# niksaz/aido1

Measured on AMD Instinct MI355X. Metric: env-steps/sec (whole node) at 4096 envs/GPU; pose/reward max-abs-err vs CPU ref, higher is better.
Workload: dtype f64 step / f32 raster + grey / u8 masks; 1 GPU; config3: 4096 envs/GPU, lane pose + 120x160 top-down render + grey frame ring + line_detector1 HSV/edge masks; map=loop_empty, envs_per_gpu=4096, global_envs=4096, repeat_actions=3, auto_reset=True, actions=U[0,1)^2 wheel velocities, resident in HBM, parallelism=env shards (1 x 4096), no collective

## Files before the change

aido1_amd/_lib.py:

```python
import ctypes
import os
import subprocess
import threading

from aido1_amd.config import DtConfig

PKG_DIR = os.path.dirname(os.path.abspath(__file__))
REPO_DIR = os.path.dirname(PKG_DIR)
LIB_PATH = os.path.join(PKG_DIR, 'libdtsim.so')
CSRC = os.path.join(PKG_DIR, 'csrc')
SOURCES = ['dtsim.hip', 'dtrender.hip', 'dtreplay.hip', 'dtactor.hip', 'dtconv.hip',
           'dtconvx.hip', 'dttrain.hip', 'dtupd.hip', 'dthead.hip']
HEADERS = ['dtsim_common.h', 'dtrender.h', 'dtsync.h', 'dtconv_common.h']
PUBLIC_HEADERS = ['dtsim.h', 'dtreplay.h', 'dtactor.h', 'dttrain.h', 'dtupd.h', 'dthead.h']
HIPCC = os.environ.get('HIPCC', '/opt/rocm/bin/hipcc')
ABI_VERSION = 14

HIP_FLAGS = ['--offload-arch=gfx950', '-O3', '-fPIC', '-shared', '-std=c++17',
             '-ffp-contract=off', '-munsafe-fp-atomics']
FILE_FLAGS = {'dtrender.hip': ['-fno-slp-vectorize']}


class DtError(RuntimeError):
    pass
# ... 83 lines not shown
                print(' '.join(cmd))

        def run(cmd):
            return subprocess.run(cmd, capture_output=True, text=True)
        with ThreadPoolExecutor(max_workers=min(8, len(jobs))) as ex:
            results = list(ex.map(run, [c for c, _ in jobs]))
        for (cmd, _), r in zip(jobs, results):
            if r.returncode != 0:
                raise DtError('hipcc failed building %s (%s):\n' % (
                    os.path.basename(path), os.path.basename(cmd[-3])) + r.stderr[-4000:])
        link = [HIPCC, '--offload-arch=gfx950', '-shared', '-fPIC', '-o', tmp] + \
            [o for _, o in jobs]
        if verbose:
            print(' '.join(link))
        r = subprocess.run(link, capture_output=True, text=True)
        if r.returncode != 0:
            raise DtError('hipcc failed linking %s:\n' % os.path.basename(path) + r.stderr[-4000:])
        os.replace(tmp, path)
    finally:
        shutil.rmtree(objdir, ignore_errors=True)
    return path


_OPTIONAL = set()

_lib = None
_lock = threading.Lock()


def bind(L):
    vp, i32, u32, u64 = ctypes.c_void_p, ctypes.c_int32, ctypes.c_uint32, ctypes.c_uint64
    i64, f64 = ctypes.c_int64, ctypes.c_double
    sig = {
        'dt_abi_version': (i32, []),
        'dt_create': (ctypes.c_int, [ctypes.POINTER(DtConfig), ctypes.POINTER(DtMap), u64, i32,
                                     i32, ctypes.POINTER(vp)]),
        'dt_destroy': (ctypes.c_int, [vp]),
        'dt_n_envs': (i32, [vp]),
        'dt_last_error': (ctypes.c_char_p, [vp]),
        'dt_seed': (ctypes.c_int, [vp, vp, u64, u32]),
        'dt_reset': (ctypes.c_int, [vp, vp, vp]),
        'dt_step': (ctypes.c_int, [vp, vp, vp, vp, vp, vp, vp, vp, vp]),
        'dt_step_masked': (ctypes.c_int, [vp, vp, vp, vp, vp, vp, vp, vp, vp, vp]),
        'dt_step_many': (ctypes.c_int, [vp, i32, vp, vp, vp, vp, vp, vp, vp]),
        'dt_seed_env': (ctypes.c_int, [vp, i32, u64]),
        'dt_lane_pos': (ctypes.c_int, [vp, vp, vp, vp]),
        'dt_render': (ctypes.c_int, [vp, vp, vp]),
        'dt_render2': (ctypes.c_int, [vp, vp, vp, vp]),
        'dt_render3': (ctypes.c_int, [vp, vp, vp, vp, vp]),
        'dt_copy_pose': (ctypes.c_int, [vp, vp, vp]),
        'dt_render_order': (ctypes.c_int, [vp, ctypes.POINTER(u32), vp, vp]),
        'dt_palette_gray': (ctypes.c_int, [ctypes.POINTER(ctypes.c_float)]),
        'dt_default_line_params': (ctypes.c_int, [vp]),
        'dt_set_line_params': (ctypes.c_int, [vp, vp]),
        'dt_line_detect': (ctypes.c_int, [vp, vp, i32, i32, i32, vp, vp, vp]),
        'dt_hough_lines': (ctypes.c_int, [vp, i32, i32, i32, i32, i32, i32, i32, vp, vp,
                                          vp]),
        'dt_line_detect_workspace': (ctypes.c_size_t, [i32, i32, i32]),
        'dt_line_detect_ws': (ctypes.c_int, [vp, vp, i32, i32, i32, vp, vp, vp,
                                             ctypes.c_size_t, vp]),
        'dt_hough_workspace': (ctypes.c_size_t, [i32, i32, i32]),
        'dt_hough_lines_ws': (ctypes.c_int, [vp, i32, i32, i32, i32, i32, i32, i32, vp, vp,
                                             vp, ctypes.c_size_t, vp]),
        'dt_get_state': (ctypes.c_int, [vp, vp, vp, vp, vp, vp, vp]),
        'dt_set_state': (ctypes.c_int, [vp, vp, vp, vp, vp, vp, vp]),
        'dt_check': (ctypes.c_int, [vp, ctypes.POINTER(u32)]),
        'dt_stats': (ctypes.c_int, [vp, ctypes.POINTER(ctypes.c_uint64), i32]),
        'dt_per_create': (ctypes.c_int, [i64, f64, i32, ctypes.POINTER(vp)]),
        'dt_per_destroy': (None, [vp]),
        'dt_per_last_error': (ctypes.c_char_p, [vp]),
        'dt_per_capacity': (i64, [vp]),
        'dt_per_len': (i64, [vp]),
        'dt_per_next_idx': (i64, [vp]),
        'dt_per_add': (ctypes.c_int, [vp, i64, vp, vp]),
        'dt_per_sample': (ctypes.c_int, [vp, i32, vp, f64, vp, vp, vp]),
# ... 149 lines not shown
```

aido1_amd/csrc/dthandle.h:

```cpp
#pragma once
#include <string>

#include "dtrender.h"
#include "dtsim_common.h"

struct StepCfg {
  int32_t repeat, frame_skip, action_mode, clip, speed_measured, auto_reset;
  uint32_t max_steps, max_env_steps, max_spawn_attempts;
  double reward_scale;
};

struct dt_handle {
  int device = 0;
  int n = 0;
  dt_config cfg{};
  dt::Geo geo{};
  StepCfg sc{};
  dt::MapDev map{};
  void* map_buf = nullptr;
  dt::State st{};
  void* st_buf = nullptr;
  size_t lds_bytes = 0;
  uint32_t env_base = 0;
  dt_line_params line_params{};
  dr::LineDev line{};
  void* mark_buf = nullptr;
  int32_t n_yellow = 0, n_white = 0;
  void* render_spill = nullptr;
  void* render_sched = nullptr;
  uint32_t render_launches = 0;
  hipEvent_t render_done = nullptr;
  hipStream_t render_stream = nullptr;
  bool render_pending = false;
  std::string err;
};

struct DevGuard {
  int prev = -1;
  explicit DevGuard(int device) {
    if (hipGetDevice(&prev) == hipSuccess && prev != device) {
      if (hipSetDevice(device) != hipSuccess) prev = -1;
    } else {
      prev = -1;
    }
  }
  ~DevGuard() {
    if (prev >= 0) (void)hipSetDevice(prev);
  }
  DevGuard(const DevGuard&) = delete;
  DevGuard& operator=(const DevGuard&) = delete;
// ... 16 lines not shown
```

aido1_amd/csrc/dtrender.h:

```cpp
#pragma once
#pragma clang fp contract(off)

#include <hip/hip_runtime.h>
#include <stdint.h>

#include "../../include/dtsim.h"

namespace dr {

constexpr int H = DT_OBS_H, W = DT_OBS_W, NPIX = H * W;
constexpr int kThreads = 256;
constexpr float kRes = 0.01f;
constexpr float kInvRes = 100.0f;

enum : uint8_t { PAL_FLOOR = 0, PAL_OFFROAD = 1, PAL_ROAD = 2, PAL_RED = 3, PAL_YELLOW = 4,
                 PAL_WHITE = 7, PAL_N = 8 };
__host__ __device__ constexpr uint32_t rgb_pack(uint32_t r, uint32_t g, uint32_t b) {
  return b | (g << 8) | (r << 16);
}
constexpr uint32_t kYellowRgb = rgb_pack(255, 230, 0);
constexpr uint32_t kPalette[PAL_N] = {
    rgb_pack(0, 0, 0),
    rgb_pack(72, 132, 52),
    rgb_pack(56, 56, 60),
// ... 71 lines not shown
  const int c0 = c > 0 ? c - 1 : 0, c2 = c < wid - 1 ? c + 1 : wid - 1;
  const uint32_t p00 = fetch(r0, c0), p01 = fetch(r0, c), p02 = fetch(r0, c2);
  const uint32_t p10 = fetch(r, c0), p12 = fetch(r, c2);
  const uint32_t p20 = fetch(r2, c0), p21 = fetch(r2, c), p22 = fetch(r2, c2);
  mag = -1;
  dx = dy = 0;
#pragma unroll
  for (int ch = 0; ch < 3; ++ch) {
    const int sh = 8 * ch;
    const int a00 = (p00 >> sh) & 255, a01 = (p01 >> sh) & 255, a02 = (p02 >> sh) & 255;
    const int a10 = (p10 >> sh) & 255, a12 = (p12 >> sh) & 255;
    const int a20 = (p20 >> sh) & 255, a21 = (p21 >> sh) & 255, a22 = (p22 >> sh) & 255;
    const int gx = (a02 + 2 * a12 + a22) - (a00 + 2 * a10 + a20);
    const int gy = (a20 + 2 * a21 + a22) - (a00 + 2 * a01 + a02);
    const int m = (gx < 0 ? -gx : gx) + (gy < 0 ? -gy : gy);
    if (m > mag) {
      mag = m;
      dx = gx;
      dy = gy;
    }
  }
}

__device__ inline uint8_t nms_dir(int dx, int dy) {
  constexpr int TG22 = 13573;
  const int x = dx < 0 ? -dx : dx;
  const int y = (dy < 0 ? -dy : dy) << 15;
  const int tg22x = x * TG22;
  if (y < tg22x) return 0;
  const int tg67x = tg22x + (x << 16);
  if (y > tg67x) return 1;
  return ((dx ^ dy) < 0) ? 3 : 2;
}

}
```

aido1_amd/csrc/dtrender.hip:

```cpp
#include <math.h>
#include <stdlib.h>
#include <string.h>

#include <vector>

#include "dthandle.h"

namespace {

using namespace dr;

#ifdef DTSIM_STAMPS
__device__ unsigned long long g_renstamps[4096 * 24];
__device__ inline unsigned ren_hw_id() {
  unsigned v;
  asm volatile("s_getreg_b32 %0, hwreg(HW_REG_HW_ID)" : "=s"(v));
  return v;
}
__device__ inline unsigned ren_xcc_id() {
  unsigned v;
  asm volatile("s_getreg_b32 %0, hwreg(HW_REG_XCC_ID)" : "=s"(v));
  return v;
}
#define RENSTAMP(i, v)                                                              \
// ... 45 lines not shown
        double dx, dz;
        bez_host(cp, (double)k / kSegs, px[k], pz[k], dx, dz);
        const double n = sqrt(dx * dx + dz * dz);
        rx[k] = (0.0 - dz) / n;
        rz[k] = dx / n;
      }
      for (int w = 0; w < kWhiteW; ++w) {
        const double o = kWhiteOff * ts + (2 * w - (kWhiteW - 1)) * kHalfStep;
        for (int k = 0; k < kSegs; ++k)
          white.push_back(make_float4((float)(px[k] + o * rx[k]), (float)(pz[k] + o * rz[k]),
                                      (float)(px[k + 1] + o * rx[k + 1]),
                                      (float)(pz[k + 1] + o * rz[k + 1])));
      }
      if (c != 0) continue;
      for (int w = 0; w < kYellowW; ++w) {
        const double o = kYellowOff * ts + (2 * w - (kYellowW - 1)) * kHalfStep;
        for (int k = 0; k < kSegs; k += 2)
          yellow.push_back(make_float4((float)(px[k] + o * rx[k]), (float)(pz[k] + o * rz[k]),
                                       (float)(px[k + 1] + o * rx[k + 1]),
                                       (float)(pz[k + 1] + o * rz[k + 1])));
      }
    }
  }
}

LineDev to_line_dev(const dt_line_params& p) {
  LineDev L{};
  memcpy(L.lo[0], p.hsv_white1, 3);
  memcpy(L.hi[0], p.hsv_white2, 3);
  memcpy(L.lo[1], p.hsv_yellow1, 3);
  memcpy(L.hi[1], p.hsv_yellow2, 3);
  memcpy(L.lo[2], p.hsv_red1, 3);
  memcpy(L.hi[2], p.hsv_red2, 3);
  memcpy(L.lo[3], p.hsv_red3, 3);
  memcpy(L.hi[3], p.hsv_red4, 3);
  const int k = p.dilation_kernel_size;
  const int r = k / 2;
  L.dil_r = r;
  L.dil_mask = 0;
  if (r == 0) {
    L.dil_mask = 1ull << (3 * 7 + 3);
  } else {
    const double inv_r2 = 1.0 / ((double)r * r);
    for (int i = 0; i < k; ++i) {
      const int dy = i - r;
      const int dxm = (int)lrint(r * sqrt((double)(r * r - dy * dy) * inv_r2));
// ... 105 lines not shown
      if (hyst_visit(S, hgt, wid, idx)) changed = 1;
    if (!__syncthreads_or(changed)) break;
  }
}

__device__ inline uint8_t pass_c_pixel(const PixBuf& S, const LineDev& L, int hgt, int wid, int r,
                                       int c) {
  uint8_t bits = 0;
  const int R = L.dil_r;
  for (int dy = -R; dy <= R; ++dy) {
    const int rr = r + dy;
    if ((unsigned)rr >= (unsigned)hgt) continue;
    for (int dx = -R; dx <= R; ++dx) {
      const int cc = c + dx;
      if ((unsigned)cc >= (unsigned)wid) continue;
      if (!((L.dil_mask >> ((dy + 3) * 7 + (dx + 3))) & 1ull)) continue;
      bits |= S.work[rr * wid + cc] & 7;
    }
  }
  if (S.work[r * wid + c] & B_EDGE) bits |= 8;
  return bits;
}

struct View {
  float cx, cz, dirx, dirz, rx, rz;
};

__device__ __forceinline__ int opaque_tid() {
  int t = (int)threadIdx.x;
#if DTSIM_RENDER_SEQ
  asm volatile("" : "+v"(t));
#endif
  return t;
}

#ifndef DTSIM_RENDER_SEQ
#define DTSIM_RENDER_SEQ 0
#endif
struct RenderArgs {
  const double* x;
  const double* z;
  const double* angle;
  const int8_t* kind;
  int32_t width, height;
  float inv_ts;
  double cam_fwd;
  const float4* marks;
  int32_t n_yellow, n_white;
  float* gray;
  uint8_t* index;
  int32_t slots, slot;
  const uint8_t* fresh;
  uint8_t* masks;
  uint8_t* rgb;
  uint16_t* spill;
  int32_t list_cap;
  LineDev line;
  int32_t n;
  uint32_t* sched;
  uint32_t launch;
  int32_t parts;
  int32_t slot2, slot3;
  const double* pose2;
  const double* pose3;
  const uint8_t* fresh2;
  const uint8_t* fresh3;
  uint8_t* masks2;
  uint8_t* masks3;
};

#ifndef DTSIM_MARK_PARTS
#define DTSIM_MARK_PARTS 2
#endif
#ifndef DTSIM_RENDER_THREADS
#define DTSIM_RENDER_THREADS 512
#endif
constexpr int kRenderThreads = DTSIM_RENDER_THREADS;
#ifdef DTSIM_RENDER_STOP_AT
#define RENDER_STOP(k) \
  if ((k) == DTSIM_RENDER_STOP_AT) return
#else
#define RENDER_STOP(k)
#endif
constexpr int WPR = W / 4;
constexpr int NW = NPIX / 4;
constexpr int QPR = WPR / 4;
constexpr int NQ = NW / 4;
constexpr int kListCap = 1984;
constexpr int kWeakCap = 512;
constexpr int kSegRecs = 2176;
constexpr int kSpillHalves = 5 * NW;
enum { kNSpan = 0, kNSeg = 1, kNList = 2, kNQuad = 3, kNWeak = 4, kNCnt = 8 };
constexpr uint16_t WK_MAG = 0x7FF, WK_DIR_SHIFT = 11, WK_CAND = 1 << 14, WK_EDGE = 1 << 15;

struct RenderLds {
  uint32_t img[NW];
  union {
    struct {
      uint16_t ent[4 * kListCap];
      uint16_t list[kListCap];
    } w;
    struct {
      uint2 seg[kSegRecs];
      uint16_t qlist[NQ];
    } p;
  } u;
  uint16_t weak[kWeakCap];
  uint32_t pal_swar[PAL_N];
  float pal_gray[PAL_N];
  uint32_t bits_lo, bits_hi;
  View view[3];
  int32_t cnt[kNCnt];
  int32_t env;
// ... 102 lines not shown

__device__ inline void wave_slots4(int32_t* counter, const bool want[4], int slot[4]) {
  wave_slotsN<4>(counter, want, slot);
}

__device__ inline int wave_slot1(int32_t* counter, bool want) {
  const uint64_t b = __ballot(want);
  if (b == 0) return 0;
  int base = 0;
  if ((threadIdx.x & 63) == 0) base = atomicAdd(counter, __popcll(b));
  base = __builtin_amdgcn_readlane(base, 0);
  return base + lane_prefix(b);
}

__device__ inline void wave_push4(int32_t* counter, uint16_t* list, int cap, const bool want[4],
                                  const uint16_t value[4]) {
  int slot[4];
  wave_slots4(counter, want, slot);
#pragma unroll
  for (int k = 0; k < 4; ++k)
    if (want[k] && slot[k] < cap) list[slot[k]] = value[k];
}

__device__ inline void wave_slots4x2(int32_t* counter, const bool wa[4], const bool wb[4],
                                     int sa[4], int sb[4]) {
  const uint32_t ca = (uint32_t)wa[0] + wa[1] + wa[2] + wa[3];
  const uint32_t cb = (uint32_t)wb[0] + wb[1] + wb[2] + wb[3];
  const uint64_t a0 = __ballot(ca & 1u), a1 = __ballot(ca & 2u), a2 = __ballot(ca & 4u);
  const uint64_t b0 = __ballot(cb & 1u), b1 = __ballot(cb & 2u), b2 = __ballot(cb & 4u);
  const uint32_t ta = __popcll(a0) + 2 * __popcll(a1) + 4 * __popcll(a2);
  const uint32_t tb = __popcll(b0) + 2 * __popcll(b1) + 4 * __popcll(b2);
  if ((ta | tb) == 0u) return;
  int base = 0;
  if ((threadIdx.x & 63) == 0) base = atomicAdd(counter, (int)(ta | (tb << 16)));
  base = __builtin_amdgcn_readlane(base, 0);
  int na = (base & 0xFFFF) + lane_prefix(a0) + 2 * lane_prefix(a1) + 4 * lane_prefix(a2);
  int nb = (int)((uint32_t)base >> 16) + lane_prefix(b0) + 2 * lane_prefix(b1) +
           4 * lane_prefix(b2);
#pragma unroll
  for (int k = 0; k < 4; ++k) {
    sa[k] = na;
    na += wa[k] ? 1 : 0;
    sb[k] = nb;
    nb += wb[k] ? 1 : 0;
  }
}

using lds_u32 = __attribute__((address_space(3))) uint32_t;

__device__ __forceinline__ void or_pixel(lds_u32* img, uint32_t ad, uint32_t col) {
  __hip_atomic_fetch_or(img + (ad >> 2), col << (8 * (ad & 3u)), __ATOMIC_RELAXED,
                        __HIP_MEMORY_SCOPE_WORKGROUP);
}

__device__ inline void draw_line_part(lds_u32* img, int x0, int y0, int x1, int y1, uint32_t col,
                                      int part, int parts) {
  int dx = x1 - x0, dy = y1 - y0;
  const int xsign = dx > 0 ? 1 : -1, ysign = dy > 0 ? 1 : -1;
  dx = dx < 0 ? -dx : dx;
  dy = dy < 0 ? -dy : dy;
  int xx, xy, yx, yy;
  if (dx > dy) {
    xx = xsign; xy = 0; yx = 0; yy = ysign;
  } else {
    const int t = dx; dx = dy; dy = t;
    xx = 0; xy = ysign; yx = xsign; yy = 0;
  }
  const int n = dx + 1;
  const int xa = (n * part) / parts, xb = (n * (part + 1)) / parts;
  if (xa >= xb) return;
  const int ya = dx > 0 ? (int)floorf((float)(2 * dy * xa + dx) / (float)(2 * dx)) : 0;
  int D = 2 * dy * (xa + 1) - dx - 2 * dx * ya;
  int px = x0 + xa * xx + ya * yx, py = y0 + xa * xy + ya * yy;
  int ad = py * W + px;
  const int amaj = xy * W + xx, amin = yy * W + yx;
  for (int x = xa; x < xb; ++x) {
    if ((unsigned)px < (unsigned)W && (unsigned)py < (unsigned)H) or_pixel(img, (uint32_t)ad, col);
    const bool st = D >= 0;
    px += xx + (st ? yx : 0);
    py += xy + (st ? yy : 0);
    ad += amaj + (st ? amin : 0);
    D += 2 * dy - (st ? 2 * dx : 0);
  }
}

__device__ inline int proj(float v) {
  v = floorf(v + 0.5f);
  v = v < -100000.0f ? -100000.0f : (v > 100000.0f ? 100000.0f : v);
  return (int)v;
}

__device__ inline bool project_seg(const View& V, float4 q, int& c0, int& r0, int& c1, int& r1) {
  const float ax = q.x - V.cx, az = q.y - V.cz, bx = q.z - V.cx, bz = q.w - V.cz;
  const float fa = ax * V.dirx + az * V.dirz, la = ax * V.rx + az * V.rz;
  const float fb = bx * V.dirx + bz * V.dirz, lb = bx * V.rx + bz * V.rz;
  c0 = proj(la * kInvRes + 79.5f);
  r0 = proj(119.5f - fa * kInvRes);
  c1 = proj(lb * kInvRes + 79.5f);
  r1 = proj(119.5f - fb * kInvRes);
  if ((c0 < 0 && c1 < 0) || (c0 >= W && c1 >= W) || (r0 < 0 && r1 < 0) || (r0 >= H && r1 >= H))
    return false;
  const int len = (c1 > c0 ? c1 - c0 : c0 - c1) + (r1 > r0 ? r1 - r0 : r0 - r1);
  return len <= 400;
}

__device__ inline uint2 seg_pack(int c0, int r0, int c1, int r1) {
  return make_uint2((uint32_t)(uint16_t)c0 | ((uint32_t)(uint16_t)r0 << 16),
                    (uint32_t)(uint16_t)c1 | ((uint32_t)(uint16_t)r1 << 16));
}

__device__ inline void seg_draw(lds_u32* img, uint2 v, uint32_t col, int part, int parts) {
  draw_line_part(img, (int)(int16_t)(v.x & 0xFFFFu), (int)(int16_t)(v.x >> 16),
                 (int)(int16_t)(v.y & 0xFFFFu), (int)(int16_t)(v.y >> 16), col, part, parts);
}

__device__ __forceinline__ uint32_t bg_color(const RenderLds& S, const RenderArgs& a, float fi,
                                             float fj) {
  if (fi >= 0.0f && fj >= 0.0f && fi < (float)a.width && fj < (float)a.height) {
    const int k = S.kind[__mul24((int)fj, a.width) + (int)fi];
    return k > 0 ? PAL_ROAD : (k == 0 ? PAL_OFFROAD : PAL_FLOOR);
  }
  return PAL_FLOOR;
}

__device__ inline View view_of(double x, double z, double ang, double cam_fwd) {
  double sd, cd;
// ... 441 lines not shown

__device__ __forceinline__ uint32_t sched_builder(const RenderArgs& a) {
#if DTSIM_RENDER_SEQ
  return (uint32_t)(a.n - kSchedTail);
#else
  return (uint32_t)(a.parts * a.n - kSchedTail);
#endif
}

__device__ __forceinline__ void sched_exit(const RenderArgs& a, RenderLds& S, int e) {
  if (threadIdx.x == 0) {
    const unsigned long long dt = __builtin_amdgcn_s_memtime() - S.t0;
    __hip_atomic_store(sched_cost(a) + e, dt > 0xFFFFFFFFull ? 0xFFFFFFFFu : (uint32_t)dt,
                       __ATOMIC_RELAXED, __HIP_MEMORY_SCOPE_AGENT);
  }
  if (blockIdx.x == sched_builder(a) && a.n <= kSchedMaxN) {
    __syncthreads();
    sched_build(a, S, a.launch);
  }
}

template <bool kIdx, bool kBigR>
__device__ __forceinline__ void render_env(const RenderArgs& a, RenderLds& S, int e, int half,
                                           int vi
#ifdef DTSIM_EARLY_MARKS
                                           , const float4 (&mq)[4]
#endif
) {
  const int tid = opaque_tid();
  constexpr int T = kRenderThreads;
  const LineDev& L = a.line;
  const int nmark = a.n_yellow + a.n_white;
  const bool mfast = nmark <= kMarkFast;
#ifdef DTSIM_STAMPS
  RENSTAMP(0, __builtin_amdgcn_s_memrealtime());
  RENSTAMP(2, ren_hw_id());
  RENSTAMP(3, ren_xcc_id());
#endif
  RENT(4);
  int32_t* const C = S.cnt;
  const View V = S.view[vi];
  lds_u32* const img = (lds_u32*)S.img;
#ifndef DTSIM_EARLY_MARKS
  float4 mq[4];
  if (mfast) {
#pragma unroll
    for (int k = 0; k < 4; ++k) {
      const int sidx = tid + k * T;
      mq[k] = sidx < nmark ? a.marks[sidx] : make_float4(-1e9f, -1e9f, -1e9f, -1e9f);
    }
  }
#endif

  const auto tile_f = [&](int r, int c, float& fi, float& fj) {
    const float f = (119.5f - (float)r) * kRes;
    const float bx = V.cx + f * V.dirx, bz = V.cz + f * V.dirz;
    const float l = ((float)c - 79.5f) * kRes;
    const float wx = bx + l * V.rx, wz = bz + l * V.rz;
    fi = floorf(wx * a.inv_ts);
    fj = floorf(wz * a.inv_ts);
  };
  for (int q0 = 0; q0 < NQ; q0 += T) {
    const int q = q0 + tid;
    bool want = false;
    if (q < NQ) {
      const int r = q / QPR, c0 = 16 * (q - r * QPR);
      float fi0, fj0, fi1, fj1;
      tile_f(r, c0, fi0, fj0);
      tile_f(r, c0 + 15, fi1, fj1);
      const uint32_t col0 = bg_color(S, a, fi0, fj0);
      bool uni = fi0 == fi1 && fj0 == fj1;
      if (!uni && fabsf(fi1 - fi0) + fabsf(fj1 - fj0) == 1.0f)
        uni = bg_color(S, a, fi1, fj1) == col0;
      const uint32_t wd = uni ? splat_byte(col0) : 0u;
      *reinterpret_cast<uint4*>(S.img + 4 * q) = make_uint4(wd, wd, wd, wd);
      want = !uni;
    }
    const int slot = wave_slot1(&C[kNSpan], want);
    if (want) S.u.p.qlist[slot] = (uint16_t)q;
  }
  RENT(18);
  if (mfast) {
    bool vy[4], vw[4];
    int cc0[4], rr0[4], cc1[4], rr1[4], sy[4], sw[4];
#pragma unroll
    for (int k = 0; k < 4; ++k) {
      const int sidx = tid + k * T;
      const bool v = sidx < nmark && project_seg(V, mq[k], cc0[k], rr0[k], cc1[k], rr1[k]);
      vy[k] = v && sidx < a.n_yellow;
      vw[k] = v && sidx >= a.n_yellow;
    }
    wave_slots4x2(&C[kNSeg], vy, vw, sy, sw);
#pragma unroll
    for (int k = 0; k < 4; ++k) {
      if (vy[k]) S.u.p.seg[sy[k]] = seg_pack(cc0[k], rr0[k], cc1[k], rr1[k]);
      if (vw[k]) S.u.p.seg[kSegRecs - 1 - sw[k]] = seg_pack(cc0[k], rr0[k], cc1[k], rr1[k]);
    }
  }
  __syncthreads();
  RENT(5);
  RENDER_STOP(1);

  constexpr int kParts = DTSIM_MARK_PARTS;
  {
    const int nspan = C[kNSpan];
    const int ny = mfast ? (C[kNSeg] & 0xFFFF) : 0, nw = mfast ? (int)((uint32_t)C[kNSeg] >> 16) : 0;
    const int nbg = 4 * nspan, items = nbg + kParts * (ny + nw);
    for (int i = tid; i < items; i += T) {
      if (i < nbg) {
        const int q = S.u.p.qlist[i >> 2];
        const int r = q / QPR, c = 16 * (q - r * QPR) + 4 * (i & 3);
        float fi[4], fj[4];
        tile_f(r, c, fi[0], fj[0]);
        tile_f(r, c + 3, fi[3], fj[3]);
        const uint32_t col0 = bg_color(S, a, fi[0], fj[0]);
        uint32_t wd;
        if (fi[0] == fi[3] && fj[0] == fj[3]) {
          wd = splat_byte(col0);
        } else {
          tile_f(r, c + 1, fi[1], fj[1]);
          tile_f(r, c + 2, fi[2], fj[2]);
          wd = col0;
#pragma unroll
          for (int k = 1; k < 4; ++k) wd |= bg_color(S, a, fi[k], fj[k]) << (8 * k);
        }
        __hip_atomic_fetch_or(img + 4 * q + (i & 3), wd, __ATOMIC_RELAXED,
                              __HIP_MEMORY_SCOPE_WORKGROUP);
      } else {
        const int j = i - nbg, sidx = j / kParts;
        const bool yel = sidx < ny;
        seg_draw(img, S.u.p.seg[yel ? sidx : kSegRecs - 1 - (sidx - ny)], yel ? PAL_YELLOW : PAL_WHITE,
                 j - sidx * kParts, kParts);
      }
    }
  }
  if (!mfast) {
    int listed = 0;
#pragma unroll 1
    for (int colr = 0; colr < 2; ++colr) {
      const float4* seg = colr == 0 ? a.marks : a.marks + a.n_yellow;
      const int nseg = colr == 0 ? a.n_yellow : a.n_white;
      const uint32_t col = colr == 0 ? PAL_YELLOW : PAL_WHITE;
#pragma unroll 1
      for (int b0 = 0; b0 < nseg; b0 += kMarkFast) {
        bool vis[4];
        int cc0[4], rr0[4], cc1[4], rr1[4], slot[4];
#pragma unroll
        for (int k = 0; k < 4; ++k) {
          const int sidx = b0 + tid + k * T;
          const bool in = tid + k * T < kMarkFast && sidx < nseg;
          const float4 q = in ? seg[sidx] : make_float4(-1e9f, -1e9f, -1e9f, -1e9f);
          vis[k] = in && project_seg(V, q, cc0[k], rr0[k], cc1[k], rr1[k]);
        }
        wave_slots4(&C[kNSeg], vis, slot);
#pragma unroll
        for (int k = 0; k < 4; ++k)
          if (vis[k]) S.u.p.seg[slot[k] % kSegRecs] = seg_pack(cc0[k], rr0[k], cc1[k], rr1[k]);
        __syncthreads();
        const int end = C[kNSeg];
// ... 107 lines not shown
  const unsigned long long t16 = __builtin_amdgcn_s_memtime(), t17 = __builtin_amdgcn_s_memrealtime();
#endif
  const LineDev& L = a.line;
  if (tid < PAL_N) {
    const uint32_t p = kPalette[tid];
    S.pal_swar[tid] = swar_of(p);
    S.pal_gray[tid] = kPalGray[tid];
  }
  if (tid == 0) {
    S.bits_lo = L.pal_bits[0];
    S.bits_hi = L.pal_bits[1];
#pragma unroll
    for (int i = 0; i < kNCnt; ++i) S.cnt[i] = 0;
  }
  for (int i = tid; i < a.width * a.height; i += kRenderThreads) S.kind[i] = a.kind[i];
#if DTSIM_RENDER_SEQ
  const int nseq = a.parts, blk = (int)blockIdx.x, half0 = 0;
#else
  const int nseq = 1;
  const int blk = (int)blockIdx.x / a.parts;
  const int half0 = (int)blockIdx.x - blk * a.parts;
#endif
  int e = blk;
#ifdef DTSIM_EARLY_MARKS
  float4 mq[4];
  {
    const int nmark = a.n_yellow + a.n_white;
#pragma unroll
    for (int k = 0; k < 4; ++k) {
      const int sidx = tid + k * kRenderThreads;
      mq[k] = nmark <= kMarkFast && sidx < nmark ? a.marks[sidx]
                                                 : make_float4(-1e9f, -1e9f, -1e9f, -1e9f);
    }
  }
#endif
  if (tid >= 64 && tid < 64 + nseq) {
    const int vi = tid - 64, half = half0 + vi;
    if (a.sched) {
      const int p = sched_perm(a, a.launch)[blk];
      e = (unsigned)p < (unsigned)a.n ? p : blk;
    }
    if (vi == 0) {
      S.env = e;
      S.t0 = __builtin_amdgcn_s_memtime();
    }
    if (half) {
      const size_t n = (size_t)a.n;
      const double* ps = half == 1 ? a.pose2 : a.pose3;
      S.view[vi] = view_of(ps[e], ps[n + e], ps[2 * n + e], a.cam_fwd);
    } else {
      S.view[vi] = view_of(a.x[e], a.z[e], a.angle[e], a.cam_fwd);
    }
  }
  __syncthreads();
  e = __builtin_amdgcn_readfirstlane(S.env);
#ifdef DTSIM_STAMPS
  RENSTAMP(16, t16);
  RENSTAMP(17, t17);
#endif
  for (int vi = 0; vi < nseq; ++vi) {
    if (vi > 0) {
      __syncthreads();
      if (tid < kNCnt) S.cnt[tid] = 0;
      __syncthreads();
    }
    render_env<kIdx, kBigR>(a, S, e, half0 + vi, vi
#ifdef DTSIM_EARLY_MARKS
               , mq
#endif
    );
  }
  if (a.sched) sched_exit(a, S, e);
}

__global__ __launch_bounds__(kThreads) void line_detect_kernel(LineDev L, const uint8_t* bgr,
                                                               int hgt, int wid, uint8_t* masks,
                                                               uint8_t* hsv) {
  __shared__ __attribute__((aligned(16))) uint32_t src[NPIX];
  __shared__ __attribute__((aligned(16))) Lds S;
  const int e = blockIdx.x, np = hgt * wid;
  const PixBuf B{S.mag, S.work, S.sdiv, S.hdiv};
  const uint8_t* in = bgr + (size_t)e * np * 3;
  for (int p = threadIdx.x; p < np; p += blockDim.x)
    src[p] = (uint32_t)in[3 * p] | ((uint32_t)in[3 * p + 1] << 8) | ((uint32_t)in[3 * p + 2] << 16);
  load_tables(S.sdiv, S.hdiv);
  __syncthreads();
  const auto fetch = [&](int r, int c) -> uint32_t { return src[r * wid + c]; };
  for (int p = threadIdx.x; p < np; p += blockDim.x) {
    const int r = p / wid, c = p - r * wid;
    pass_a_pixel(fetch, B, L, hgt, wid, r, c);
    if (hsv) {
      int h, s, v;
      const uint32_t q = src[p];
// ... 247 lines not shown
      }
    }
    if (good) {
      if (lane == 0) {
        out[4 * nlines] = ex[0];
        out[4 * nlines + 1] = ey[0];
        out[4 * nlines + 2] = ex[1];
        out[4 * nlines + 3] = ey[1];
      }
      if (++nlines >= max_lines) {
        truncated = count > 1;
        break;
      }
    }
    overflow = __ballot(overflow) != 0;
  }
  const bool any_over = __ballot(overflow) != 0;
  if (lane == 0) counts[e] = any_over ? -1 : (truncated ? -2 : nlines);
}

}

int dt_render_init(dt_handle* h, const dt_map* map) {
  std::vector<float4> yellow, white;
  build_marks(map, h->cfg.road_tile_size, yellow, white);
  h->n_yellow = (int)yellow.size();
  h->n_white = (int)white.size();
  std::vector<float4> all(yellow);
  all.insert(all.end(), white.begin(), white.end());
  if (!all.empty()) {
    if (hipMalloc(&h->mark_buf, all.size() * sizeof(float4)) != hipSuccess) {
      h->err = "hipMalloc(markings) failed";
      return DT_E_HIP;
    }
    if (hipMemcpy(h->mark_buf, all.data(), all.size() * sizeof(float4), hipMemcpyHostToDevice) !=
        hipSuccess) {
      h->err = "hipMemcpy(markings) failed";
      return DT_E_HIP;
    }
  }
  dt_default_line_params(&h->line_params);
  h->line = to_line_dev(h->line_params);
  if (hipMalloc(&h->render_spill, (size_t)h->n * kSpillHalves * sizeof(uint16_t)) != hipSuccess) {
    h->err = "hipMalloc(render spill) failed";
    return DT_E_HIP;
  }
  std::vector<uint32_t> sch((size_t)kSchedHead + 3 * (size_t)h->n, 0u);
  for (int k = 0; k < 2; ++k)
    for (int i = 0; i < h->n; ++i) sch[kSchedHead + (size_t)h->n * (1 + k) + i] = (uint32_t)i;
  if (hipMalloc(&h->render_sched, sch.size() * sizeof(uint32_t)) != hipSuccess ||
      hipMemcpy(h->render_sched, sch.data(), sch.size() * sizeof(uint32_t),
                hipMemcpyHostToDevice) != hipSuccess) {
// ... 1 lines not shown
    return DT_E_HIP;
  }
  return DT_OK;
}

void dt_render_free(dt_handle* h) {
  if (h->mark_buf) (void)hipFree(h->mark_buf);
  h->mark_buf = nullptr;
  if (h->render_spill) (void)hipFree(h->render_spill);
  h->render_spill = nullptr;
  if (h->render_sched) (void)hipFree(h->render_sched);
  h->render_sched = nullptr;
  if (h->render_done) (void)hipEventDestroy(h->render_done);
  h->render_done = nullptr;
}

extern "C" {

#ifdef DTSIM_STAMPS
int dt_diag_renstamps(unsigned long long* out) {
  return hipMemcpyFromSymbol(out, HIP_SYMBOL(g_renstamps), sizeof(g_renstamps)) == hipSuccess ? 0 : -1;
}
#endif

int dt_default_line_params(dt_line_params* p) {
  if (!p) return DT_E_ARG;
  const uint8_t v[8][3] = {{0, 0, 150},    {180, 60, 255},  {25, 140, 100}, {45, 255, 255},
                           {0, 140, 100},  {15, 255, 255},  {165, 140, 100}, {180, 255, 255}};
  memcpy(p->hsv_white1, v[0], 3);
  memcpy(p->hsv_white2, v[1], 3);
  memcpy(p->hsv_yellow1, v[2], 3);
  memcpy(p->hsv_yellow2, v[3], 3);
  memcpy(p->hsv_red1, v[4], 3);
  memcpy(p->hsv_red2, v[5], 3);
  memcpy(p->hsv_red3, v[6], 3);
  memcpy(p->hsv_red4, v[7], 3);
  p->dilation_kernel_size = 3;
  p->canny_lo = 80;
  p->canny_hi = 200;
  return DT_OK;
}

int dt_set_line_params(dt_handle* h, const dt_line_params* p) {
  if (!h || !p) return DT_E_ARG;
  if (p->dilation_kernel_size < 1 || p->dilation_kernel_size > 7 ||
      (p->dilation_kernel_size & 1) == 0) {
// ... 51 lines not shown
  if ((io->gray || io->index) &&
      (io->gray_slots < 1 || io->gray_slot < 0 || io->gray_slot >= io->gray_slots)) {
    h->err = "dt_render: gray_slot out of range";
    return DT_E_ARG;
  }
  if (io->list_cap < 0) {
    h->err = "dt_render: list_cap must be >= 0";
    return DT_E_ARG;
  }
  DevGuard dg(h->device);
  RenderArgs a{};
  const size_t n = (size_t)h->n;
  a.x = io->pose ? io->pose : h->st.x;
  a.z = io->pose ? io->pose + n : h->st.z;
  a.angle = io->pose ? io->pose + 2 * n : h->st.angle;
  a.kind = h->map.kind;
  a.width = h->map.width;
  a.height = h->map.height;
  a.inv_ts = (float)(1.0 / h->cfg.road_tile_size);
  a.cam_fwd = h->cfg.camera_forward_dist;
  a.marks = (const float4*)h->mark_buf;
  a.n_yellow = h->n_yellow;
  a.n_white = h->n_white;
  a.gray = io->gray;
  a.index = io->index;
  a.slots = io->gray_slots < 1 ? 1 : io->gray_slots;
  a.slot = io->gray_slot;
  a.fresh = io->fresh;
  a.masks = io->masks;
  a.rgb = io->rgb;
  a.line = h->line;
  a.n = h->n;
  a.spill = (uint16_t*)h->render_spill;
#ifndef DTSIM_NO_SCHED
  hipStreamCaptureStatus cap = hipStreamCaptureStatusNone;
  if (hipStreamIsCapturing((hipStream_t)stream, &cap) != hipSuccess)
    cap = hipStreamCaptureStatusNone;
  a.sched = h->n > kSchedTail && cap == hipStreamCaptureStatusNone
                ? (uint32_t*)h->render_sched : nullptr;
  if (a.sched && h->render_pending && (hipStream_t)stream != h->render_stream) {
    if (!h->render_done)
      HIP_OR_FAIL(h, hipEventCreateWithFlags(&h->render_done,
                                             hipEventDisableTiming | hipEventDisableSystemFence));
    if (hipEventRecord(h->render_done, h->render_stream) == hipSuccess) {
      HIP_OR_FAIL(h, hipStreamWaitEvent((hipStream_t)stream, h->render_done, 0));
    } else {
// ... 195 lines not shown
```

aido1_amd/render.py:

```python
import ctypes

import torch

from aido1_amd import _lib

H, W = 120, 160
NPIX = H * W
MASK_WHITE, MASK_YELLOW, MASK_RED, MASK_EDGES = range(4)

RENDER_BYTES_PER_ENV = 4 * NPIX + 4 * NPIX + 24
RENDER_BYTES_PER_FRESH = 2 * 4 * NPIX
RENDER_INDEX_BYTES_PER_ENV = NPIX + 4 * NPIX + 24
RENDER_INDEX_BYTES_PER_FRESH = 2 * NPIX

_GRAY = {}


def palette_gray(device):
    key = str(torch.device(device))
    if key not in _GRAY:
        buf = (ctypes.c_float * 8)()
        if _lib.lib().dt_palette_gray(buf) != 0:
            raise _lib.DtError('dt_palette_gray failed')
        _GRAY[key] = torch.tensor(list(buf), dtype=torch.float32, device=device)
    return _GRAY[key]


def decode_index(frames):
    if frames.dtype != torch.uint8:
        raise ValueError('decode_index: uint8 palette-index frames expected')
    return palette_gray(frames.device)[frames.long()]


def as_gray(frames):
    return decode_index(frames) if frames.dtype == torch.uint8 else frames


class LineParams(ctypes.Structure):
    _fields_ = [('hsv_white1', ctypes.c_uint8 * 3), ('hsv_white2', ctypes.c_uint8 * 3),
                ('hsv_yellow1', ctypes.c_uint8 * 3), ('hsv_yellow2', ctypes.c_uint8 * 3),
                ('hsv_red1', ctypes.c_uint8 * 3), ('hsv_red2', ctypes.c_uint8 * 3),
                ('hsv_red3', ctypes.c_uint8 * 3), ('hsv_red4', ctypes.c_uint8 * 3),
                ('dilation_kernel_size', ctypes.c_int32),
                ('canny_lo', ctypes.c_double), ('canny_hi', ctypes.c_double)]

    @classmethod
    def default(cls):
        p = cls()
# ... 253 lines not shown
```

include/dtsim.h:

```cpp
#ifndef AIDO1_AMD_DTSIM_H
#define AIDO1_AMD_DTSIM_H

#include <stdint.h>

#ifdef __cplusplus
extern "C" {
#endif

#define DT_ABI_VERSION 14

#define DT_OK 0
#define DT_E_ARG (-1)
#define DT_E_HIP (-2)
#define DT_E_SPAWN (-3)
#define DT_E_NODEV (-4)

#define DT_ACTION_WHEELS 0
#define DT_ACTION_TANH 1
#define DT_ACTION_STEERING 2

#define DT_TILE_EMPTY (-1)
#define DT_TILE_OFFROAD 0
#define DT_TILE_STRAIGHT 1
#define DT_TILE_CURVE_LEFT 2
// ... 98 lines not shown
typedef struct dt_render_io {
  float* gray;
  int32_t gray_slots;
  int32_t gray_slot;
  const uint8_t* fresh;
  uint8_t* masks;
  uint8_t* rgb;
  const double* pose;
  int32_t list_cap;
  uint8_t* index;
} dt_render_io;

int dt_palette_gray(float* gray8);

int dt_render(dt_handle* h, const dt_render_io* io, void* stream);

int dt_render2(dt_handle* h, const dt_render_io* io_a, const dt_render_io* io_b, void* stream);

int dt_render3(dt_handle* h, const dt_render_io* io_a, const dt_render_io* io_b,
               const dt_render_io* io_c, void* stream);

int dt_render_order(dt_handle* h, uint32_t* launches, uint32_t* cost, int32_t* order);

int dt_copy_pose(dt_handle* h, double* pose, void* stream);
int dt_set_line_params(dt_handle* h, const dt_line_params* p);

size_t dt_line_detect_workspace(int32_t n, int32_t height, int32_t width);
int dt_line_detect_ws(const dt_line_params* p, const uint8_t* bgr, int32_t n, int32_t height,
                      int32_t width, uint8_t* masks, uint8_t* hsv, void* workspace,
                      size_t workspace_bytes, void* stream);
int dt_line_detect(const dt_line_params* p, const uint8_t* bgr, int32_t n, int32_t height,
                   int32_t width, uint8_t* masks, uint8_t* hsv, void* stream);

int dt_hough_lines(const uint8_t* edge, int32_t n, int32_t height, int32_t width,
                   int32_t threshold, int32_t min_line_length, int32_t max_line_gap,
                   int32_t max_lines, int32_t* lines, int32_t* counts, void* stream);
size_t dt_hough_workspace(int32_t n, int32_t height, int32_t width);
int dt_hough_lines_ws(const uint8_t* edge, int32_t n, int32_t height, int32_t width,
                      int32_t threshold, int32_t min_line_length, int32_t max_line_gap,
                      int32_t max_lines, int32_t* lines, int32_t* counts, void* workspace,
                      size_t workspace_bytes, void* stream);

int dt_get_state(dt_handle* h, double* x, double* z, double* angle, uint32_t* step_count,
                 uint32_t* env_step, uint32_t* episode);
int dt_set_state(dt_handle* h, const double* x, const double* z, const double* angle,
                 const uint32_t* step_count, const uint32_t* env_step, const uint32_t* episode);
// ... 10 lines not shown
```

Baseline: 88.14 million env-steps/s.

## Cull lane-marking segments by bounding-circle groups before per-segment projection

```diff
diff --git a/aido1_amd/_lib.py b/aido1_amd/_lib.py
--- a/aido1_amd/_lib.py
+++ b/aido1_amd/_lib.py
@@ -129,7 +129,7 @@
     return path
 
 
-_OPTIONAL = set()
+_OPTIONAL = {'dt_marks_probe'}
 
 _lib = None
 _lock = threading.Lock()
@@ -158,6 +158,8 @@
         'dt_copy_pose': (ctypes.c_int, [vp, vp, vp]),
         'dt_render_order': (ctypes.c_int, [vp, ctypes.POINTER(u32), vp, vp]),
         'dt_palette_gray': (ctypes.c_int, [ctypes.POINTER(ctypes.c_float)]),
+        'dt_marks_probe': (ctypes.c_int, [ctypes.POINTER(DtMap), f64, f64, i32, vp, vp, vp, vp,
+                                          ctypes.POINTER(i64), ctypes.POINTER(i32)]),
         'dt_default_line_params': (ctypes.c_int, [vp]),
         'dt_set_line_params': (ctypes.c_int, [vp, vp]),
         'dt_line_detect': (ctypes.c_int, [vp, vp, i32, i32, i32, vp, vp, vp]),
diff --git a/aido1_amd/csrc/dthandle.h b/aido1_amd/csrc/dthandle.h
--- a/aido1_amd/csrc/dthandle.h
+++ b/aido1_amd/csrc/dthandle.h
@@ -25,7 +25,7 @@
   dt_line_params line_params{};
   dr::LineDev line{};
   void* mark_buf = nullptr;
-  int32_t n_yellow = 0, n_white = 0;
+  int32_t n_yellow = 0, n_white = 0, n_groups = 0;
   void* render_spill = nullptr;
   void* render_sched = nullptr;
   uint32_t render_launches = 0;
diff --git a/aido1_amd/csrc/dtrender.h b/aido1_amd/csrc/dtrender.h
--- a/aido1_amd/csrc/dtrender.h
+++ b/aido1_amd/csrc/dtrender.h
@@ -117,6 +117,47 @@
   }
 }
 
+struct View {
+  float cx, cz, dirx, dirz, rx, rz;
+};
+
+__host__ __device__ inline int proj(float v) {
+  v = floorf(v + 0.5f);
+#ifdef __HIP_DEVICE_COMPILE__
+  int i;
+  asm("v_cvt_i32_f32 %0, %1" : "=v"(i) : "v"(v));
+  return i < -100000 ? -100000 : (i > 100000 ? 100000 : i);
+#else
+  if (v != v) return 0;
+  v = v < -100000.0f ? -100000.0f : (v > 100000.0f ? 100000.0f : v);
+  return (int)v;
+#endif
+}
+
+__host__ __device__ inline bool project_seg(const View& V, float4 q, int& c0, int& r0, int& c1,
+                                            int& r1) {
+  const float ax = q.x - V.cx, az = q.y - V.cz, bx = q.z - V.cx, bz = q.w - V.cz;
+  const float fa = ax * V.dirx + az * V.dirz, la = ax * V.rx + az * V.rz;
+  const float fb = bx * V.dirx + bz * V.dirz, lb = bx * V.rx + bz * V.rz;
+  c0 = proj(la * kInvRes + 79.5f);
+  r0 = proj(119.5f - fa * kInvRes);
+  c1 = proj(lb * kInvRes + 79.5f);
+  r1 = proj(119.5f - fb * kInvRes);
+  if ((c0 < 0 && c1 < 0) || (c0 >= W && c1 >= W) || (r0 < 0 && r1 < 0) || (r0 >= H && r1 >= H))
+    return false;
+  const int len = (c1 > c0 ? c1 - c0 : c0 - c1) + (r1 > r0 ? r1 - r0 : r0 - r1);
+  return len <= 400;
+}
+
+constexpr int kGroupSegs = 8;
+constexpr float kCullMargin = 0.02f, kCullRel = 4e-6f;
+__host__ __device__ inline bool group_off(const View& V, float gx, float gz, float gr) {
+  const float ax = gx - V.cx, az = gz - V.cz;
+  const float f = ax * V.dirx + az * V.dirz, l = ax * V.rx + az * V.rz;
+  const float R = gr + (kCullMargin + kCullRel * (fabsf(f) + fabsf(l)));
+  return f + R < 0.0f || f - R > 1.2f || l + R < -0.8f || l - R > 0.8f;
+}
+
 __device__ inline uint8_t nms_dir(int dx, int dy) {
   constexpr int TG22 = 13573;
   const int x = dx < 0 ? -dx : dx;
diff --git a/aido1_amd/csrc/dtrender.hip b/aido1_amd/csrc/dtrender.hip
--- a/aido1_amd/csrc/dtrender.hip
+++ b/aido1_amd/csrc/dtrender.hip
@@ -91,6 +91,45 @@
       }
     }
   }
+}
+
+void build_groups(const std::vector<float4>& yellow, const std::vector<float4>& white,
+                  std::vector<float4>& all, std::vector<float4>& groups) {
+  all = yellow;
+  all.insert(all.end(), white.begin(), white.end());
+  groups.clear();
+  if (yellow.size() % kGroupSegs || white.size() % kGroupSegs) return;
+  for (size_t g = 0; g < all.size() / kGroupSegs; ++g) {
+    const float4* q = all.data() + g * kGroupSegs;
+    double x0 = q[0].x, x1 = x0, z0 = q[0].y, z1 = z0;
+    for (int k = 0; k < kGroupSegs; ++k) {
+      x0 = fmin(x0, fmin((double)q[k].x, (double)q[k].z));
+      x1 = fmax(x1, fmax((double)q[k].x, (double)q[k].z));
+      z0 = fmin(z0, fmin((double)q[k].y, (double)q[k].w));
+      z1 = fmax(z1, fmax((double)q[k].y, (double)q[k].w));
+    }
+    const float cx = (float)(0.5 * (x0 + x1)), cz = (float)(0.5 * (z0 + z1));
+    double r = 0.0;
+    for (int k = 0; k < kGroupSegs; ++k) {
+      r = fmax(r, hypot((double)q[k].x - cx, (double)q[k].y - cz));
+      r = fmax(r, hypot((double)q[k].z - cx, (double)q[k].w - cz));
+    }
+    float rf = (float)r;
+    if ((double)rf <= r) rf = nextafterf(rf, INFINITY);
+    groups.push_back(make_float4(cx, cz, rf, 0.0f));
+  }
+}
+
+View view_host(double x, double z, double ang, double cam_fwd) {
+  const double sd = sin(ang), cd = cos(ang);
+  View v;
+  v.cx = (float)(x + cam_fwd * cd);
+  v.cz = (float)(z + cam_fwd * (-sd));
+  v.dirx = (float)cd;
+  v.dirz = -(float)sd;
+  v.rx = (float)sd;
+  v.rz = (float)cd;
+  return v;
 }
 
 LineDev to_line_dev(const dt_line_params& p) {
@@ -242,10 +281,6 @@
   return bits;
 }
 
-struct View {
-  float cx, cz, dirx, dirz, rx, rz;
-};
-
 __device__ __forceinline__ int opaque_tid() {
   int t = (int)threadIdx.x;
 #if DTSIM_RENDER_SEQ
@@ -267,6 +302,8 @@
   double cam_fwd;
   const float4* marks;
   int32_t n_yellow, n_white;
+  const float4* groups;
+  int32_t n_groups;
   float* gray;
   uint8_t* index;
   int32_t slots, slot;
@@ -309,6 +346,11 @@
 constexpr int kListCap = 1984;
 constexpr int kWeakCap = 512;
 constexpr int kSegRecs = 2176;
+#ifndef DTSIM_SEG_CAP
+#define DTSIM_SEG_CAP kSegRecs
+#endif
+constexpr int kSegCap = DTSIM_SEG_CAP;
+static_assert(kSegCap <= kSegRecs, "the record area");
 constexpr int kSpillHalves = 5 * NW;
 enum { kNSpan = 0, kNSeg = 1, kNList = 2, kNQuad = 3, kNWeak = 4, kNCnt = 8 };
 constexpr uint16_t WK_MAG = 0x7FF, WK_DIR_SHIFT = 11, WK_CAND = 1 << 14, WK_EDGE = 1 << 15;
@@ -457,28 +499,14 @@
     if (want[k] && slot[k] < cap) list[slot[k]] = value[k];
 }
 
-__device__ inline void wave_slots4x2(int32_t* counter, const bool wa[4], const bool wb[4],
-                                     int sa[4], int sb[4]) {
-  const uint32_t ca = (uint32_t)wa[0] + wa[1] + wa[2] + wa[3];
-  const uint32_t cb = (uint32_t)wb[0] + wb[1] + wb[2] + wb[3];
-  const uint64_t a0 = __ballot(ca & 1u), a1 = __ballot(ca & 2u), a2 = __ballot(ca & 4u);
-  const uint64_t b0 = __ballot(cb & 1u), b1 = __ballot(cb & 2u), b2 = __ballot(cb & 4u);
-  const uint32_t ta = __popcll(a0) + 2 * __popcll(a1) + 4 * __popcll(a2);
-  const uint32_t tb = __popcll(b0) + 2 * __popcll(b1) + 4 * __popcll(b2);
-  if ((ta | tb) == 0u) return;
+__device__ inline void wave_slot1x2(int32_t* counter, bool wa, bool wb, int& sa, int& sb) {
+  const uint64_t ba = __ballot(wa), bb = __ballot(wb);
+  if ((ba | bb) == 0) return;
   int base = 0;
-  if ((threadIdx.x & 63) == 0) base = atomicAdd(counter, (int)(ta | (tb << 16)));
+  if ((threadIdx.x & 63) == 0) base = atomicAdd(counter, __popcll(ba) | (__popcll(bb) << 16));
   base = __builtin_amdgcn_readlane(base, 0);
-  int na = (base & 0xFFFF) + lane_prefix(a0) + 2 * lane_prefix(a1) + 4 * lane_prefix(a2);
-  int nb = (int)((uint32_t)base >> 16) + lane_prefix(b0) + 2 * lane_prefix(b1) +
-           4 * lane_prefix(b2);
-#pragma unroll
-  for (int k = 0; k < 4; ++k) {
-    sa[k] = na;
-    na += wa[k] ? 1 : 0;
-    sb[k] = nb;
-    nb += wb[k] ? 1 : 0;
-  }
+  sa = (base & 0xFFFF) + lane_prefix(ba);
+  sb = (int)((uint32_t)base >> 16) + lane_prefix(bb);
 }
 
 using lds_u32 = __attribute__((address_space(3))) uint32_t;
@@ -517,26 +545,6 @@
     ad += amaj + (st ? amin : 0);
     D += 2 * dy - (st ? 2 * dx : 0);
   }
-}
-
-__device__ inline int proj(float v) {
-  v = floorf(v + 0.5f);
-  v = v < -100000.0f ? -100000.0f : (v > 100000.0f ? 100000.0f : v);
-  return (int)v;
-}
-
-__device__ inline bool project_seg(const View& V, float4 q, int& c0, int& r0, int& c1, int& r1) {
-  const float ax = q.x - V.cx, az = q.y - V.cz, bx = q.z - V.cx, bz = q.w - V.cz;
-  const float fa = ax * V.dirx + az * V.dirz, la = ax * V.rx + az * V.rz;
-  const float fb = bx * V.dirx + bz * V.dirz, lb = bx * V.rx + bz * V.rz;
-  c0 = proj(la * kInvRes + 79.5f);
-  r0 = proj(119.5f - fa * kInvRes);
-  c1 = proj(lb * kInvRes + 79.5f);
-  r1 = proj(119.5f - fb * kInvRes);
-  if ((c0 < 0 && c1 < 0) || (c0 >= W && c1 >= W) || (r0 < 0 && r1 < 0) || (r0 >= H && r1 >= H))
-    return false;
-  const int len = (c1 > c0 ? c1 - c0 : c0 - c1) + (r1 > r0 ? r1 - r0 : r0 - r1);
-  return len <= 400;
 }
 
 __device__ inline uint2 seg_pack(int c0, int r0, int c1, int r1) {
@@ -1024,16 +1032,10 @@
 
 template <bool kIdx, bool kBigR>
 __device__ __forceinline__ void render_env(const RenderArgs& a, RenderLds& S, int e, int half,
-                                           int vi
-#ifdef DTSIM_EARLY_MARKS
-                                           , const float4 (&mq)[4]
-#endif
-) {
+                                           int vi, float4 gc) {
   const int tid = opaque_tid();
   constexpr int T = kRenderThreads;
   const LineDev& L = a.line;
-  const int nmark = a.n_yellow + a.n_white;
-  const bool mfast = nmark <= kMarkFast;
 #ifdef DTSIM_STAMPS
   RENSTAMP(0, __builtin_amdgcn_s_memrealtime());
   RENSTAMP(2, ren_hw_id());
@@ -1043,16 +1045,29 @@
   int32_t* const C = S.cnt;
   const View V = S.view[vi];
   lds_u32* const img = (lds_u32*)S.img;
-#ifndef DTSIM_EARLY_MARKS
-  float4 mq[4];
-  if (mfast) {
-#pragma unroll
-    for (int k = 0; k < 4; ++k) {
-      const int sidx = tid + k * T;
-      mq[k] = sidx < nmark ? a.marks[sidx] : make_float4(-1e9f, -1e9f, -1e9f, -1e9f);
-    }
-  }
-#endif
+
+  constexpr int kWaves = T / 64, kPerRound = 64 / kGroupSegs;
+  const int lane = tid & 63;
+  const int G = (a.n_yellow | a.n_white) < 65536 ? a.n_groups : 0;
+  const int gyel = a.n_yellow / kGroupSegs;
+  int nk = 0, mine = 0;
+  const auto cull = [&](int g, const float4& c) {
+    const bool keep = g < G && !group_off(V, c.x, c.y, c.z);
+    const uint64_t kb = __ballot(keep);
+    nk = __popcll(kb);
+    const int below = lane_prefix(kb);
+    mine = __builtin_amdgcn_ds_permute((keep ? below : nk + lane - below) << 2, g);
+  };
+  const auto seg_of = [&](int r, int& gid) -> float4 {
+    const int s = kPerRound * r + lane / kGroupSegs;
+    gid = __builtin_amdgcn_ds_bpermute((s & 63) << 2, mine);
+    gid = s < nk ? gid : -1;
+    return gid >= 0 ? a.marks[gid * kGroupSegs + lane % kGroupSegs] : make_float4(0.f, 0.f, 0.f, 0.f);
+  };
+  const int g0 = (tid >> 6) + kWaves * lane;
+  cull(g0, gc);
+  int gid0, gid1;
+  const float4 mq0 = seg_of(0, gid0), mq1 = seg_of(1, gid1);
 
   const auto tile_f = [&](int r, int c, float& fi, float& fj) {
     const float f = (119.5f - (float)r) * kRes;
@@ -1082,31 +1097,42 @@
     if (want) S.u.p.qlist[slot] = (uint16_t)q;
   }
   RENT(18);
-  if (mfast) {
-    bool vy[4], vw[4];
-    int cc0[4], rr0[4], cc1[4], rr1[4], sy[4], sw[4];
-#pragma unroll
-    for (int k = 0; k < 4; ++k) {
-      const int sidx = tid + k * T;
-      const bool v = sidx < nmark && project_seg(V, mq[k], cc0[k], rr0[k], cc1[k], rr1[k]);
-      vy[k] = v && sidx < a.n_yellow;
-      vw[k] = v && sidx >= a.n_yellow;
-    }
-    wave_slots4x2(&C[kNSeg], vy, vw, sy, sw);
-#pragma unroll
-    for (int k = 0; k < 4; ++k) {
-      if (vy[k]) S.u.p.seg[sy[k]] = seg_pack(cc0[k], rr0[k], cc1[k], rr1[k]);
-      if (vw[k]) S.u.p.seg[kSegRecs - 1 - sw[k]] = seg_pack(cc0[k], rr0[k], cc1[k], rr1[k]);
-    }
+  const auto emit = [&](int gid, const float4& q) {
+    int c0, r0, c1, r1, sy = 0, sw = 0;
+    const bool v = gid >= 0 && project_seg(V, q, c0, r0, c1, r1);
+    const bool vy = v && gid < gyel, vw = v && gid >= gyel;
+    wave_slot1x2(&C[kNSeg], vy, vw, sy, sw);
+    const int at = vy ? sy : kSegRecs - 1 - sw;
+    if (v && (vy ? sy : sw) < kSegRecs) S.u.p.seg[at] = seg_pack(c0, r0, c1, r1);
+  };
+  if (nk > 0) {
+    emit(gid0, mq0);
+    if (nk > kPerRound) emit(gid1, mq1);
+  }
+#pragma unroll 1
+  for (int gb = 0, r = 2;; r = 0) {
+#pragma unroll 1
+    for (; kPerRound * r < nk; ++r) {
+      int gid;
+      const float4 q = seg_of(r, gid);
+      emit(gid, q);
+    }
+    gb += 64 * kWaves;
+    if (gb >= G) break;
+    const int g = gb + g0;
+    cull(g, g < G ? a.groups[g] : make_float4(0.f, 0.f, 0.f, 0.f));
   }
   __syncthreads();
   RENT(5);
   RENDER_STOP(1);
 
   constexpr int kParts = DTSIM_MARK_PARTS;
+  bool mover;
   {
     const int nspan = C[kNSpan];
-    const int ny = mfast ? (C[kNSeg] & 0xFFFF) : 0, nw = mfast ? (int)((uint32_t)C[kNSeg] >> 16) : 0;
+    int ny = C[kNSeg] & 0xFFFF, nw = (int)((uint32_t)C[kNSeg] >> 16);
+    mover = G == 0 || ny + nw > kSegCap;
+    if (mover) ny = nw = 0;
     const int nbg = 4 * nspan, items = nbg + kParts * (ny + nw);
     for (int i = tid; i < items; i += T) {
       if (i < nbg) {
@@ -1136,7 +1162,10 @@
       }
     }
   }
-  if (!mfast) {
+  if (mover) {
+    __syncthreads();
+    if (tid == 0) C[kNSeg] = 0;
+    __syncthreads();
     int listed = 0;
 #pragma unroll 1
     for (int colr = 0; colr < 2; ++colr) {
@@ -1290,18 +1319,8 @@
   const int half0 = (int)blockIdx.x - blk * a.parts;
 #endif
   int e = blk;
-#ifdef DTSIM_EARLY_MARKS
-  float4 mq[4];
-  {
-    const int nmark = a.n_yellow + a.n_white;
-#pragma unroll
-    for (int k = 0; k < 4; ++k) {
-      const int sidx = tid + k * kRenderThreads;
-      mq[k] = nmark <= kMarkFast && sidx < nmark ? a.marks[sidx]
-                                                 : make_float4(-1e9f, -1e9f, -1e9f, -1e9f);
-    }
-  }
-#endif
+  const int g0 = (tid >> 6) + (kRenderThreads / 64) * (tid & 63);
+  const float4 gc = g0 < a.n_groups ? a.groups[g0] : make_float4(0.f, 0.f, 0.f, 0.f);
   if (tid >= 64 && tid < 64 + nseq) {
     const int vi = tid - 64, half = half0 + vi;
     if (a.sched) {
@@ -1332,11 +1351,7 @@
       if (tid < kNCnt) S.cnt[tid] = 0;
       __syncthreads();
     }
-    render_env<kIdx, kBigR>(a, S, e, half0 + vi, vi
-#ifdef DTSIM_EARLY_MARKS
-               , mq
-#endif
-    );
+    render_env<kIdx, kBigR>(a, S, e, half0 + vi, vi, gc);
   }
   if (a.sched) sched_exit(a, S, e);
 }
@@ -1630,12 +1645,13 @@
 }
 
 int dt_render_init(dt_handle* h, const dt_map* map) {
-  std::vector<float4> yellow, white;
+  std::vector<float4> yellow, white, all, groups;
   build_marks(map, h->cfg.road_tile_size, yellow, white);
+  build_groups(yellow, white, all, groups);
   h->n_yellow = (int)yellow.size();
   h->n_white = (int)white.size();
-  std::vector<float4> all(yellow);
-  all.insert(all.end(), white.begin(), white.end());
+  h->n_groups = (int)groups.size();
+  all.insert(all.end(), groups.begin(), groups.end());
   if (!all.empty()) {
     if (hipMalloc(&h->mark_buf, all.size() * sizeof(float4)) != hipSuccess) {
       h->err = "hipMalloc(markings) failed";
@@ -1683,6 +1699,36 @@
   return hipMemcpyFromSymbol(out, HIP_SYMBOL(g_renstamps), sizeof(g_renstamps)) == hipSuccess ? 0 : -1;
 }
 #endif
+
+int dt_marks_probe(const dt_map* map, double tile_size, double cam_fwd, int32_t n, const double* x,
+                   const double* z, const double* angle, int32_t* kept, int64_t* lost,
+                   int32_t* n_groups) {
+  if (!map || !map->kind || !map->curve_start || !map->curves || n < 0 ||
+      (n > 0 && (!x || !z || !angle)))
+    return DT_E_ARG;
+  std::vector<float4> yellow, white, all, groups;
+  build_marks(map, tile_size, yellow, white);
+  build_groups(yellow, white, all, groups);
+  if (n_groups) *n_groups = (int32_t)groups.size();
+  int64_t nlost = 0;
+  for (int32_t i = 0; i < n; ++i) {
+    const View V = view_host(x[i], z[i], angle[i], cam_fwd);
+    int32_t nkept = 0;
+    for (size_t g = 0; g < groups.size(); ++g) {
+      if (!group_off(V, groups[g].x, groups[g].y, groups[g].z)) {
+        ++nkept;
+        continue;
+      }
+      for (int k = 0; k < kGroupSegs; ++k) {
+        int c0, r0, c1, r1;
+        nlost += project_seg(V, all[g * kGroupSegs + k], c0, r0, c1, r1) ? 1 : 0;
+      }
+    }
+    if (kept) kept[i] = nkept;
+  }
+  if (lost) *lost = nlost;
+  return DT_OK;
+}
 
 int dt_default_line_params(dt_line_params* p) {
   if (!p) return DT_E_ARG;
@@ -1780,6 +1826,8 @@
   a.marks = (const float4*)h->mark_buf;
   a.n_yellow = h->n_yellow;
   a.n_white = h->n_white;
+  a.groups = a.marks + (h->n_yellow + h->n_white);
+  a.n_groups = h->n_groups;
   a.gray = io->gray;
   a.index = io->index;
   a.slots = io->gray_slots < 1 ? 1 : io->gray_slots;
diff --git a/aido1_amd/render.py b/aido1_amd/render.py
--- a/aido1_amd/render.py
+++ b/aido1_amd/render.py
@@ -24,6 +24,29 @@
             raise _lib.DtError('dt_palette_gray failed')
         _GRAY[key] = torch.tensor(list(buf), dtype=torch.float32, device=device)
     return _GRAY[key]
+
+
+def marks_probe(tile_map, x, z, angle, cam_fwd=None):
+    import numpy as np
+    from aido1_amd.config import CAMERA_FORWARD_DIST
+    arr = [np.ascontiguousarray(v, np.float64) for v in (x, z, angle)]
+    n = len(arr[0])
+    kind = np.ascontiguousarray(tile_map.kind, np.int8)
+    start = np.ascontiguousarray(tile_map.curve_start, np.int32)
+    curves = np.ascontiguousarray(tile_map.curves, np.float64)
+    heads = np.ascontiguousarray(tile_map.headings, np.float64)
+    ptr = lambda v: v.ctypes.data_as(ctypes.c_void_p)
+    m = _lib.DtMap(tile_map.width, tile_map.height, ptr(kind), ptr(start), ptr(curves),
+                   ptr(heads), 0, None, 0, None)
+    kept = np.zeros(n, np.int32)
+    lost, groups = ctypes.c_int64(0), ctypes.c_int32(0)
+    rc = _lib.lib().dt_marks_probe(ctypes.byref(m), tile_map.tile_size,
+                                   CAMERA_FORWARD_DIST if cam_fwd is None else cam_fwd, n,
+                                   ptr(arr[0]), ptr(arr[1]), ptr(arr[2]), ptr(kept),
+                                   ctypes.byref(lost), ctypes.byref(groups))
+    if rc != 0:
+        raise _lib.DtError('dt_marks_probe failed (%d)' % rc)
+    return kept, lost.value, groups.value
 
 
 def decode_index(frames):
diff --git a/include/dtsim.h b/include/dtsim.h
--- a/include/dtsim.h
+++ b/include/dtsim.h
@@ -144,6 +144,10 @@
 
 int dt_render_order(dt_handle* h, uint32_t* launches, uint32_t* cost, int32_t* order);
 
+int dt_marks_probe(const dt_map* map, double tile_size, double cam_fwd, int32_t n, const double* x,
+                   const double* z, const double* angle, int32_t* kept, int64_t* lost,
+                   int32_t* n_groups);
+
 int dt_copy_pose(dt_handle* h, double* pose, void* stream);
 int dt_set_line_params(dt_handle* h, const dt_line_params* p);
 
```

Result: no change. 88.47 million env-steps/s (median of 6 runs) (+0.4%).
